# itsdevbear/go-avalanche

Measured on AMD Instinct MI355X. Metric: vote-record updates/sec (node·target·round) at 1/2/4/8 GPU; % HBM roofline, higher is better.
Workload: dtype u32; 1 GPU; C4: 1M nodes x 1000 targets, k=8, Bernoulli(0.8) initial acceptance, honest, sim mode; n_nodes=1000000, n_targets=1000, k=8, parallelism=single GPU

## Files before the change

### go-avalanche_amd/csrc/engine.cpp

```cpp
#include <algorithm>
#include <cstdarg>
#include <cstdio>
#include <cstring>
#include <memory>
#include <string>
#include <utility>
#include <vector>

#include "engine.h"

using namespace aveng;

namespace aveng {

static thread_local std::string g_last_error;

int fail(int code, const char* fmt, ...) {
  char buf[512];
  va_list ap;
  va_start(ap, fmt);
  vsnprintf(buf, sizeof(buf), fmt, ap);
  va_end(ap);
  g_last_error = buf;
  return code;
// ... 145 lines not shown
  e->log_cap = (uint32_t)std::min<size_t>(e->log_alloc / e->log_shards, 0xFFFFFFFFu);
  e->mlog_cap = (uint32_t)std::min<size_t>(e->mlog_alloc / e->log_shards, 0xFFFFFFFFu);
  e->dlog_cap = (uint32_t)std::min<size_t>(e->dlog_alloc / e->log_shards, 0xFFFFFFFFu);
}

int refresh_pref(av_engine* e) {
  e->facts.snapshot_written();
  AV_HIP(avk::launch_refresh_pref((uint32_t)e->pub_mode, e->planes, e->pref[e->cur], e->byz, (uint32_t)e->n0, e->NL,
                                  e->BL, e->PS, (uint32_t)e->round, e->stream));
  return AV_OK;
}

}

namespace {

avk::PlanShape plan_shape(const av_engine* e) {
  return {e->k,      e->BL,         e->N,               e->NL,       e->PS,
          e->capped, e->peer_world, e->comm != nullptr, e->pub_mode, e->any_nopoll};
}
avk::PlanKnobs plan_knobs(const av_engine* e) {
  return {e->kernel,   e->virtual_votes, e->vv_min_bl,     e->count_lazy,     e->k_hi_virtual,
          e->ref_rows, e->uni_rows,      e->ablate_gather, e->unsynced_shard, e->quiet_tiles != 0,
          e->net_quiet != 0, e->count_changed};
}
avk::RoundPlan plan_for(const av_engine* e, bool replay) {
  return avk::plan_round(e->facts, plan_shape(e), plan_knobs(e), replay);
}

int round_checks(const av_engine* e, int64_t rounds) {
  AV_CHECK(e->round + rounds - 1 - e->log_base < e->max_log_rounds(), AV_ERR_OVERFLOW,
           "StatusUpdate log spans %lld rounds: call av_fetch_updates more often", (long long)e->max_log_rounds());
  if (e->group) {
    AV_TRY(group_alive(e));
    for (const av_engine* m : e->group->members)
      if (m != e)
        AV_CHECK(m->round == e->round + (m->peer_rank < e->peer_rank ? 1 : 0), AV_ERR_UNSUPPORTED,
                 "peer group: rank %d at round %lld, rank %d at round %lld: run one round of every rank in rank "
                 "order", e->peer_rank, (long long)e->round, m->peer_rank, (long long)m->round);
  }
  AV_CHECK(e->NL == (uint32_t)e->N || e->comm != nullptr || e->peer_world > 1 || e->N == e->n1 - e->n0 ||
               e->unsynced_shard,
           AV_ERR_UNSUPPORTED,
           "node-sharded engine needs av_comm_init before running rounds");
  return AV_OK;
}

// ... 93 lines not shown
  }
  if (e->comm) {
    const size_t count = (size_t)e->NL * e->PS;
    uint32_t* out = e->pref[nb];
    ncclResult_t r = ncclAllGather(out + (size_t)e->n0 * e->PS, out, count, ncclUint32, e->comm, e->stream);
    AV_CHECK(r == ncclSuccess, AV_ERR_RCCL, "ncclAllGather: %s", ncclGetErrorString(r));
  }
  return AV_OK;
}

int launch_one_round(av_engine* e, const uint32_t* replay) {
  AV_TRY(round_checks(e, 1));
  avk::RoundPlan plan = plan_for(e, replay != nullptr);
  AV_CHECK(!plan.unsupported, AV_ERR_UNSUPPORTED,
           "the example responder and av_set_polling need M <= 4096 (uncapped)");
  AV_TRY(materialize(e, plan.wb_votes || plan.wb_cpreset, false));
  AV_TRY(materialize(e, false, plan.wb_counts));
  avk::RoundParams p = round_params(e, replay);
  p.c_preset = e->facts.c_preset ? 1u : 0u;
  p.vv = plan.vv ? 1u : 0u;
  p.vv_uniform = plan.vv_uniform ? 1u : 0u;
  p.fresh = plan.fresh ? 1u : 0u;
  p.klazy = plan.klazy ? 1u : 0u;
  p.kconsume = plan.kconsume ? 1u : 0u;
  p.hivirt = plan.hivirt ? 1u : 0u;
  const bool sweep = plan.kernel == avk::RoundKernel::Sweep;
  const int nb = av_engine::nxt(e->cur);
  fill_push_params(e, sweep && !replay, nb, p);
  AV_TRY(fill_row_params(e, plan, nb, p));
  if (plan.net_quiet_out) {
    p.nq_out = e->nq + (e->round & 1);
    p.nq_in = plan.net_quiet_in ? e->nq + ((e->round & 1) ^ 1) : nullptr;
    p.nq_rounds = e->nq + 2;
    p.nq_group = e->nq_group;
    p.nq_front = e->nq_front;
  }
  if (e->warm_pref && sweep) {
    if (!e->touch_sink) AV_HIP(e->touch_sink.alloc(16));
    AV_HIP(avk::launch_touch(p.pref_prev, (size_t)e->N * e->PS * 4u, e->touch_sink, e->stream));
    AV_HIP(avk::launch_touch(p.pref_in, (size_t)e->N * e->PS * 4u, e->touch_sink, e->stream));
  }
  hipEvent_t ev0 = nullptr, ev1 = nullptr;
  AV_TRY(timing_begin(e, &ev0, &ev1));
  if (p.push_n && e->masked) {
    AV_TRY(need_combine(e, e->round / avk::kNeedWin));
    AV_TRY(need_draw_ahead(e, e->round / avk::kNeedWin + 1));
// ... 377 lines not shown
constexpr PlainOption opt(const char* n, bool av_engine::*m) { return {n, kBool, 0, 1, m, nullptr, nullptr}; }
constexpr PlainOption opt(const char* n, uint32_t av_engine::*m, OptKind kd = kBool, int64_t lo = 0, int64_t hi = 1) {
  return {n, kd, lo, hi, nullptr, m, nullptr};
}
constexpr PlainOption opt(const char* n, int av_engine::*m, OptKind kd, int64_t lo, int64_t hi) {
  return {n, kd, lo, hi, nullptr, nullptr, m};
}

constexpr PlainOption kPlainOptions[] = {
    opt("plane_nt", &av_engine::plane_nt),
    opt("uniform_rows", &av_engine::uni_rows),
    opt("ref_rows", &av_engine::ref_rows),
    opt("virtual_votes", &av_engine::virtual_votes),
    opt("vv_min_bl", &av_engine::vv_min_bl, kReject, 1, (1ll << 31) - 1),
    opt("kernel", &av_engine::kernel, kReject, 1, 2),
    opt("store_policy", &av_engine::store_policy, kReject, 0, 3),
    opt("settled_fast", &av_engine::settled_fast),
    opt("settled_lean", &av_engine::settled_lean),
    opt("wave_runs", &av_engine::wave_runs),
    opt("sweep_nopipe", &av_engine::sweep_nopipe),
    opt("uni_merge", &av_engine::uni_merge, kReject, 1, 16),
    opt("uni_votes", &av_engine::uni_votes),
    opt("quiet_tiles", &av_engine::quiet_tiles),
    opt("net_quiet", &av_engine::net_quiet),
    opt("net_quiet_group", &av_engine::nq_group, kReject, 1, 16),
    opt("net_quiet_front", &av_engine::nq_front),
    opt("wave_dense", &av_engine::wave_dense, kReject, 0, 64),
    opt("tile_draw", &av_engine::tile_draw, kReject, 0, 1),
    opt("materialize_run", &av_engine::mat_run, kReject, 1, 64),
    opt("c_preset", &av_engine::c_preset),
    opt("replay_fuse", &av_engine::replay_fuse, kReject, 0, 4096),
    opt("replay_fast", &av_engine::replay_fast),
    opt("dropin_fast", &av_engine::dropin_fast),
    opt("admit_map", &av_engine::admit_map, kReject, 0, 2),
    opt("push_defer", &av_engine::push_defer),
    opt("push_store", &av_engine::push_store, kReject, 0, 2),
    opt("census_blocks", &av_engine::census_blocks, kReject, 0, 65536),
    opt("copy_blocks", &av_engine::copy_blocks, kReject, 0, 4096),
    opt("enc_buckets", &av_engine::enc_buckets, kReject, 1, 1ll << 30),
    opt("count_changed", &av_engine::count_changed),
    opt("round_marker", &av_engine::round_marker),
    opt("warm_pref", &av_engine::warm_pref),
    opt("unsynced_shard", &av_engine::unsynced_shard),
    opt("ablate_gather", &av_engine::ablate_gather),
    opt("ablate_phase", &av_engine::ablate_phase, kClamp, 0, 31),
    opt("ablate_emit", &av_engine::ablate_emit, kClamp, 0, 3),
// ... 180 lines not shown
```

### go-avalanche_amd/csrc/engine.h

```cpp
#pragma once

#include <hip/hip_runtime.h>
#include <rccl/rccl.h>

#include <algorithm>
#include <cstdint>
#include <cstdlib>
#include <thread>
#include <utility>
#include <vector>

#pragma GCC visibility push(default)
#include "../../include/avhip.h"
#pragma GCC visibility pop
#include "engine_mem.h"
#include "kernels.h"
#include "round_plan.h"

namespace aveng {
int fail(int code, const char* fmt, ...) __attribute__((format(printf, 2, 3)));
inline int oom_or_hip(hipError_t he) { return he == hipErrorOutOfMemory ? AV_ERR_OOM : AV_ERR_HIP; }
}

#define AV_HIP(call)                                                                                           \
// ... 137 lines not shown
  uint32_t mat_run = 1;
  uint32_t census_blocks = 0;
  bool masked = false;
  uint32_t segs = 1;
  avmem::DevBuf<uint8_t> need_mine;
  avmem::DevBuf<uint8_t> needmask;
  avmem::DevBuf<uint8_t> stale;
  uint32_t* needin = nullptr;
  avmem::DevBuf<uint32_t> needin_own;
  avk::PeerPtrs peer_needin{};
  int64_t need_ready = -1;
  int64_t need_pushed = -1;
  avmem::Stream need_stream;
  avmem::Event need_free, need_drawn;
  int64_t need_drawn_w = -1;
  avmem::DevBuf<unsigned long long> changed;
  bool count_changed = false;
  int64_t rflag_clear_round = 0;

  uint32_t dense_min = 0;
  uint32_t wave_dense = 0;
  uint32_t uni_votes = 1;
  uint32_t quiet_tiles = 1;
  uint32_t net_quiet = 1;
  uint32_t nq_group = 16;
  uint32_t nq_front = 1;
  avmem::DevBuf<uint32_t> nq;
  int32_t pub_mode = 0;
  avmem::DevBuf<uint32_t> readd;
  avmem::DevBuf<uint32_t> died_out;
  std::vector<uint32_t> nopoll_host;
  avmem::DevBuf<uint32_t> nopoll;
  bool any_nopoll = false;
  std::vector<int64_t> proc_round;
  avmem::DevBuf<void> fetch_scratch;
  avmem::DevBuf<unsigned long long> digest;
  avmem::PinnedBuf<void> dropin_host;
  avmem::PinnedBuf<void> stage[2];
  avmem::Event stage_ev[2];
  bool dropin_fast = true;
  uint32_t admit_map = 0;
  avmem::DevBuf<uint32_t> enc_err;
  avmem::DevBuf<uint64_t> enc_tot;
  uint32_t enc_buckets = 1u << 26;
  uint32_t copy_blocks = 0;
  static constexpr int kSlots = 3;
// ... 75 lines not shown
```

### go-avalanche_amd/csrc/kernels.h

```cpp
#pragma once

#include <hip/hip_runtime.h>
#include <stdint.h>

#include <type_traits>

namespace avk {

constexpr int kPlanes = 25;
constexpr int kPV = 0, kPC = 8, kPA = 16, kPK = 17;
constexpr uint32_t kLogShards = 1024;
constexpr uint32_t kCtrStride = 32;
constexpr uint32_t kMaxPoll = 4096;
constexpr int kMaxK = 16;
constexpr int kMaxPeers = 15;

__host__ __device__ constexpr size_t replay_groups(int k) { return (size_t)((k + 1) / 2); }
__host__ __device__ inline size_t replay_words(uint32_t Lpad, int k) { return replay_groups(k) * 4u * Lpad; }
__host__ __device__ inline size_t replay_idx(uint32_t g, int k, int j, int c) {
  return (((size_t)(g >> 6) * replay_groups(k) + (size_t)(j >> 1)) * 64u + (g & 63u)) * 4u + (size_t)((j & 1) * 2 + c);
}

__host__ __device__ constexpr uint32_t pref_stride(uint32_t BL) {
  return BL > 32u ? (BL + 31u) / 32u * 32u : (BL <= 1u ? 1u : 1u << (32 - __builtin_clz(BL - 1u)));
}

constexpr uint32_t kPendAllLive = 0x80000000u;
constexpr uint32_t kHiVirt = 0x40000000u;
__host__ __device__ inline uint32_t real_mask(uint32_t tn, uint32_t b) {
  const uint32_t rem = tn > b * 32u ? tn - b * 32u : 0u;
  return rem >= 32u ? ~0u : ((1u << rem) - 1u);
}
constexpr uint32_t kVStale = 1u, kVUniform = 2u, kVMask = 3u, kCAll = 4u;

inline void bl_divider(uint32_t d, uint32_t& magic, uint32_t& sh1, uint32_t& sh2) {
  uint32_t l = 0;
  while ((1ull << l) < d) ++l;
  magic = (uint32_t)((((1ull << l) - d) << 32) / d + 1);
  sh1 = l < 1 ? l : 1;
  sh2 = l > 1 ? l - 1 : 0;
}

__host__ __device__ constexpr uint32_t dense_words(uint32_t k) { return (k + 5u) / 2u; }
__host__ __device__ constexpr uint32_t dense_min(uint32_t k) { return dense_words(k); }

constexpr uint32_t kMedS4Died = 1u << 8;
__host__ __device__ constexpr uint32_t med_rec_words() { return 4u; }

__host__ __device__ inline uint64_t pack_update(uint32_t round_rel, uint32_t node, uint32_t slot,
                                                uint32_t target, uint32_t status, uint32_t round_shift) {
  return ((uint64_t)round_rel << round_shift) | ((uint64_t)node << 28) | ((uint64_t)slot << 24) |
         ((uint64_t)target << 2) | (uint64_t)status;
}

constexpr uint32_t kDropUnknown = 1u << 29, kDropYes = 1u << 30, kDropCons = 1u << 31, kDropTl = (1u << 22) - 1u;
__host__ __device__ inline uint32_t dropin_word(int64_t tl, bool local, uint32_t err) {
// ... 81 lines not shown

  uint32_t* uni_out;
  const uint32_t* uni_in;
  const uint32_t* uni_prev;
  uint32_t uni_world, uni_rank, uni_off;
  uint32_t uni_merge;
  uint32_t uni_post;

  uint32_t fresh;
  uint32_t tn;
  uint32_t hivirt;
  uint32_t tpw;
  uint32_t settled_fast;
  uint32_t lean;
  uint32_t bl_log2;
  uint32_t nopipe;
  uint32_t pub_mode;
  uint32_t* readd;
  uint32_t* died_out;
  const uint32_t* nopoll;
  uint32_t dense_min;
  uint32_t uni_votes;
  uint32_t quiet_tiles;
  uint32_t* nq_out;
  const uint32_t* nq_in;
  uint32_t* nq_rounds;
  uint32_t nq_group;
  uint32_t nq_front;
  uint32_t wave_dense;
  uint32_t c_preset;
};

template <int MAXK, int K = 1, typename F>
hipError_t dispatch_k(int k, F&& f) {
  if constexpr (K <= MAXK) {
    return k == K ? f(std::integral_constant<int, K>{}) : dispatch_k<MAXK, K + 1>(k, f);
  } else {
    return hipErrorInvalidValue;
  }
}

struct InitParams {
  uint32_t* planes;
  uint32_t* pref;
  const uint32_t* byz;
  uint64_t seed;
// ... 157 lines not shown
```

### go-avalanche_amd/csrc/round_plan.h

```cpp
#pragma once

#include <algorithm>
#include <cstdint>

namespace avk {

enum class RoundKernel : int {
  Sweep,
  Node,
  FirstGen,
};

enum class SweepMode : int { Replay, Ablate, Fresh, Warm, Check };

struct PlanShape {
  int k;
  uint32_t BL;
  int64_t N;
  uint32_t NL, PS;
  bool capped;
  int peer_world;
  bool has_comm;
  int32_t pub_mode;
  bool any_nopoll;
};

struct PlanKnobs {
  int kernel;
  bool virtual_votes;
  uint32_t vv_min_bl;
  bool count_lazy, k_hi_virtual, ref_rows, uni_rows, ablate_gather, unsynced_shard;
  bool quiet_tiles = true, net_quiet = true, count_changed = false;
};

struct RoundPlan {
  bool unsupported;
  RoundKernel kernel;
  SweepMode mode;
  int k;
  bool replay, capped;
  bool fresh;
  bool warm;
  bool vv;
  bool vv_uniform;
  bool klazy;
  bool kconsume;
  bool hivirt;
  bool exact_pass;
  bool wb_votes, wb_counts;
  bool wb_cpreset;
  bool ref_rows, uni_rows;
  bool net_quiet_out, net_quiet_in;
};

struct RecordFacts {
  bool c_monotone = true;
  bool warm_all = false;
  bool fresh = false;
  int count_bound = 127;
  bool c_preset = false;
  bool v_stale = false;
  bool k_pend = false;
  bool rflag_ok[3] = {false, false, false};
  bool uni_ok[3] = {false, false, false};
  bool nq_ok = false;

  void snapshot_written() {
    rflag_ok[0] = rflag_ok[1] = rflag_ok[2] = false;
    uni_ok[0] = uni_ok[1] = uni_ok[2] = false;
    nq_ok = false;
  }
  void init(bool records_created, bool preset = false) {
    snapshot_written();
    warm_all = false;
    count_bound = -6;
// ... 72 lines not shown
                                                                : RoundKernel::FirstGen;
  const bool ones = f.c_monotone && f.warm_all;
  r.fresh = f.fresh && sweep && !replay && !o.ablate_gather;
  r.warm = sweep && !replay && ones && !o.ablate_gather && !r.fresh;
  r.mode = replay            ? SweepMode::Replay
           : o.ablate_gather ? SweepMode::Ablate
           : r.fresh         ? SweepMode::Fresh
           : ones            ? SweepMode::Warm
                             : SweepMode::Check;
  r.vv = o.virtual_votes && s.k == 8 && (r.warm || r.fresh);
  r.vv_uniform = r.vv && s.BL < o.vv_min_bl;
  r.klazy = o.count_lazy && r.warm && s.k == 8 && f.count_bound < 120;
  r.kconsume = !r.klazy && f.k_pend && r.warm && s.k == 8;
  r.hivirt = o.k_hi_virtual && s.k == 8;
  r.exact_pass = f.count_bound >= 120;
  r.wb_votes = !r.vv && f.v_stale;
  r.wb_counts = !r.klazy && !r.kconsume && f.k_pend;
  r.wb_cpreset = f.c_preset && !r.fresh;
  const bool tagged = sweep && s.k == 8 && !replay && !s.has_comm && !o.ablate_gather;
  r.ref_rows = o.ref_rows && tagged && 64 % s.BL == 0;
  r.uni_rows = o.uni_rows && tagged && (s.NL == (uint32_t)s.N || s.peer_world > 1 || o.unsynced_shard);
  r.net_quiet_out = o.quiet_tiles && o.net_quiet && r.klazy && sweep && !o.count_changed && s.peer_world <= 1 && !s.has_comm;
  r.net_quiet_in = r.net_quiet_out && f.nq_ok;
  return r;
}

inline bool plans_c_preset(const PlanShape& s, const PlanKnobs& o) {
  RecordFacts f;
  f.init(true);
  const RoundPlan r = plan_round(f, s, o, false);
  return r.fresh && !r.unsupported;
}

struct SweepGrid {
  uint32_t grid, run;
};
inline SweepGrid sweep_grid(uint32_t tiles, uint32_t blocks) {
  const uint32_t need = (uint32_t)(((uint64_t)tiles + 3u) / 4u);
  const uint32_t grid = std::max(1u, blocks ? std::min(blocks, need) : need);
  const uint64_t waves = (uint64_t)grid * 4u;
  return {grid, (uint32_t)((tiles + waves - 1u) / waves)};
}
inline uint64_t sweep_run_waves(uint32_t tiles, uint32_t blocks) {
  const uint64_t run = std::max(1u, sweep_grid(tiles, blocks).run);
  return std::max<uint64_t>(1, (tiles + run - 1u) / run);
}
// ... 3 lines not shown
```

### go-avalanche_amd/csrc/round_sweep.hip

```cpp
#include <hip/hip_runtime.h>

#include <algorithm>

#include "kernels.h"
#include "round_common.h"
#include "round_plan.h"
#include "round_slots.h"

#ifndef AVK_ABLATE_PHASE
#define AVK_ABLATE_PHASE 0
#endif
#ifndef AVK_PUB_PRELOAD
#define AVK_PUB_PRELOAD 0
#endif

namespace avk {
namespace {

constexpr bool kAblatePhase = AVK_ABLATE_PHASE != 0;

struct SweepAcc {
  uint32_t applied = 0, died = 0, lane_bytes = 0;
  uint32_t reread = 0;
  uint32_t emitted_bytes = 0, updates = 0;
// ... 112 lines not shown
  uint32_t kw;
  uint32_t C[WARM ? 1 : 8];
  uint32_t uref;
  uint32_t old;
  uint32_t w[K];
  uint32_t cw[REPLAY ? K : 1];
};

struct WaveDraw {
  const uint32_t* sdc;
  const uint32_t* sdp;
  unsigned long long badc, badp;
  uint32_t fofs;
  uint32_t nlA, t0, nn;
  unsigned long long flagok;
  uint32_t meta;
  bool pair, ok;
};

__device__ __forceinline__ uint32_t meta_of(const WaveDraw& wd, uint32_t tile) {
  return (uint32_t)__builtin_amdgcn_readlane((int)wd.meta, (int)(tile - wd.t0));
}

__device__ __forceinline__ uint32_t at_byte(const uint32_t* base, uint32_t off) {
  return *reinterpret_cast<const uint32_t*>(reinterpret_cast<const char*>(base) + off);
}

struct LaneIdx {
  uint32_t g, gc, nl, b, node;
  bool active;
};

__device__ __forceinline__ LaneIdx lane_idx(const RoundParams& p, uint32_t tile, uint32_t lane) {
  LaneIdx x;
  x.g = tile * 64u + lane;
  x.active = x.g < p.L;
  x.gc = x.active ? x.g : p.L - 1u;
  x.nl = div_bl(p, x.gc);
  x.b = x.gc - x.nl * p.BL;
  x.node = p.n0 + x.nl;
  return x;
}

constexpr uint32_t kUniVotes = 1u, kUniPrev = 2u;
template <int K, bool REPLAY, bool WARM, int POL, bool ABLATE, bool VVM = false, bool FRESH = false, bool CC = true>
__device__ __forceinline__ void load_tile(const RoundParams& p, uint32_t tile, uint32_t lane,
                                          TileIn<K, REPLAY, WARM>& in, const WaveDraw* wd = nullptr,
                                          uint32_t uflags = 0u) {
  const LaneIdx x = lane_idx(p, tile, lane);
  const uint32_t* const tp = p.planes + (size_t)tile * (kPlanes * 64u);
  const u32x4* const grp = reinterpret_cast<const u32x4*>(tp) + lane;
  constexpr bool VV = VVM && WARM && !REPLAY && K == 8;
  const bool meta = VV && wd && wd->t0 <= tile && tile - wd->t0 < 64u && p.tpw;
  const uint32_t raw = VV && p.vv ? (meta ? (meta_of(*wd, tile) >> 8) & 0xFFu : uni(p.vstale[tile])) : 0u;
  in.stale = raw & kVMask;
  in.cflag = raw & kCAll;
  in.kw = 0u;
  if constexpr (FRESH) {
    const uint32_t rem = p.tn - x.b * 32u;
    const uint32_t real = rem >= 32u ? ~0u : ((1u << rem) - 1u);
    in.v0 = in.v1 = in.k0 = u32x4{0u, 0u, 0u, 0u};
    in.k1 = u32x4{0u, 0u, 0u, ~real};
#pragma unroll
    for (int i = 0; i < (WARM ? 1 : 8); ++i) in.C[i] = 0u;
  } else {
    if (!in.stale) {
      in.v0 = ld4<POL>(grp);
      in.v1 = ld4<POL>(grp + 64);
    }
    if constexpr (VV) {
      if (p.klazy || p.kconsume) in.kw = meta ? meta_of(*wd, tile) & (kPendAllLive | kHiVirt | 0xFFu) : uni(p.kpend[tile]);
    }
    if (kAblatePhase && VV && (p.ablate_phase & 2u)) {
      in.k0 = u32x4{lane, 0u, 0u, 0u};
      in.k1 = u32x4{0u, 0u, 0u, ~real_mask(p.tn, x.b)};
    } else if (!(in.kw & kPendAllLive) || !p.klazy) {
      in.k0 = ld4<POL>(grp + 128);
      if (in.kw & kHiVirt)
        in.k1 = u32x4{0u, 0u, 0u, ~real_mask(p.tn, x.b)};
// ... 78 lines not shown
#pragma unroll
    for (int j = 0; j < K; ++j) in.w[j] = at_byte(p.pref_in, rows[j] + bo);
  }
}

__device__ __forceinline__ uint8_t ref_tag(uint32_t snapshot_round) { return (uint8_t)(0x80u | (snapshot_round & 0x7Fu)); }

__device__ __forceinline__ void ref_flag_store(const RoundParams& p, uint32_t lane, bool active, uint32_t b,
                                               uint32_t node, uint32_t pub, uint32_t ref) {
  const uint64_t eq = __ballot(!active || pub == ref);
  const uint32_t s0 = lane - b;
  const uint64_t seg = (p.BL >= 64u ? ~0ull : ((1ull << p.BL) - 1ull)) << (s0 & 63u);
  if (active && b == 0u) {
    const uint8_t f = (eq & seg) == seg ? ref_tag(p.round + 1u) : 0u;
    if (p.push_n && p.rflag_out[node] != f) {
      for (uint32_t r = 0; r < p.push_n; ++r)
        __hip_atomic_store(reinterpret_cast<uint8_t*>(peer_ptr(p.push_dst, r)) + p.rflag_off + node, f, __ATOMIC_RELAXED,
                           __HIP_MEMORY_SCOPE_SYSTEM);
    }
    p.rflag_out[node] = f;
  }
}

template <int K, bool REPLAY, bool WARM, int POL, bool VVM = false, bool REF = false, bool CC = true>
__device__ __forceinline__ void process_tile(const RoundParams& p, uint32_t tile, uint32_t lane,
                                             const TileIn<K, REPLAY, WARM>& in, uint32_t extra_bytes, SweepAcc& acc,
                                             uint32_t uflags = 0u) {
  const LaneIdx x = lane_idx(p, tile, lane);
  const bool active = x.active;
  const uint32_t b = x.b, node = x.node;
  const bool nbyz = ((in.byzw >> (node & 31u)) & 1u) != 0u;
  uint32_t* const tp = p.planes + (size_t)tile * (kPlanes * 64u);
  u32x4* const grp = reinterpret_cast<u32x4*>(tp) + lane;
  const __amdgpu_buffer_rsrc_t tr = __builtin_amdgcn_make_buffer_rsrc(tp, 0, kPlanes * 64 * 4, kRsrcWord3);
  const u32x4 v0 = in.v0, v1 = in.v1;
  u32x4 k0 = in.k0, k1 = in.k1;
  uint32_t A = in.A;
  uint32_t C[8];
#pragma unroll
  for (int i = 0; i < 8; ++i) C[i] = WARM ? ~0u : in.C[WARM ? 0 : i];
  const uint32_t vmask = in.vmask;

  constexpr bool SYM = WARM && !REPLAY;
  uint32_t ys[7 + K], ns[7 + K], cwv[K];
#pragma unroll
  for (int j = 0; j < K; ++j) {
    const uint32_t cw = REPLAY ? in.cw[REPLAY ? j : 0] : ~0u;
// ... 72 lines not shown
    for (int i = 0; i < 4; ++i) {
      const uint32_t bi = ((pend >> i) & 1u) ? P0 : 0u;
      const uint32_t t = Kp[3 + i] ^ bi;
      const uint32_t si = t ^ cy;
      cy = (t & cy) | (Kp[3 + i] & bi);
      Kp[3 + i] = si;
    }
  }
  uint32_t E[K], alive = P0, applied = 0u, c[4] = {0u, 0u, 0u, 0u}, F = 0u;
  const uint32_t low3[3] = {Kp[0], Kp[1], Kp[2]};
  constexpr bool KLZ_ABLATE = VVM && WARM && !REPLAY && K == 8;
  const uint32_t nearfin = klazy ? 0u : P0 & Kp[6] & Kp[5] & Kp[4] & Kp[3];
  const bool det = __ballot(nearfin != 0u) != 0ull;
  const uint32_t A_in = A;
  bool settled = false;
  if constexpr (SYM && K == 8) {
    if (!det) {
      uint32_t agree = P0;
#pragma unroll
      for (int i = 0; i < 7 + K; ++i) agree &= ~(ys[i] ^ A);
      settled = __ballot(agree != P0) == 0ull;
    }
  }
  if (settled) {
#pragma unroll
    for (int j = 0; j < K; ++j) E[j] = 0u;
    c[3] = P0;
    applied = 8u * (uint32_t)__popc(P0);
  } else if (kAblatePhase && KLZ_ABLATE && (p.ablate_phase & 16u)) {
#pragma unroll
    for (int j = 0; j < K; ++j) E[j] = 0u;
    c[3] = P0;
    applied = 8u * (uint32_t)__popc(P0);
  } else {
    round_slots<K, SYM>(ys, ns, low3, nearfin, det, alive, A, E, c, F, applied);
  }
  bool kdefer = false;
  uint32_t pend = 0u;
  if constexpr (KL) {
    if (klazy) {
      const uint32_t c8 = c[3] & ~(c[0] | c[1] | c[2]);
      const bool lane_uniform = !active || (((F & P0) | (~c8 & P0)) == 0u);
      kdefer = __ballot(!lane_uniform) == 0ull;
      pend = in.kw & 0xFFu;
      if (!kdefer) {
        if (kunread) {
          k0 = ld4<POL>(reinterpret_cast<const u32x4*>(tp) + lane + 128);
          k1 = in.kw & kHiVirt ? u32x4{0u, 0u, 0u, ~real_mask(p.tn, b)}
                               : ld4<POL>(reinterpret_cast<const u32x4*>(tp) + lane + 192);
#pragma unroll
          for (int i = 0; i < 4; ++i) {
            Kp[i] = k0[i];
            Kp[4 + i] = k1[i];
          }
        }
        uint32_t cy = 0u;
#pragma unroll
        for (int i = 0; i < 4; ++i) {
          const uint32_t bi = ((pend >> i) & 1u) ? P0 : 0u;
// ... 31 lines not shown
    if (AVK_PUB_PRELOAD && CC && p.count_changed && !known) pre = publish_loads(p, node * p.PS + b, node - p.n0);
    if (!kdefer) {
      u32x4 o2, o3;
#pragma unroll
      for (int i = 0; i < 4; ++i) {
        o2[i] = Kp[i];
        o3[i] = Kp[4 + i];
      }
      st4<POL>(tr, grp + 128, 2048u + lane * 16u, o2);
      if (!hv) st4<POL>(tr, grp + 192, 3072u + lane * 16u, o3);
    }
    if (astore) st1<POL>(tr, tp + 1536u + lane, (1536u + lane) * 4u, A);
    const uint32_t prow = node * p.PS + b;
    const uint32_t pub = nbyz ? byz_pattern(p.round + 1u) : A;
    if (p.uni_out) acc.umis |= pub != in.uref ? 1u : 0u;
    publish<POL, CC>(p, prow, pub, nbyz ? byz_pattern(p.round - 2u) : pub, acc, known, node - p.n0, acc.qslot, &pre);
  }
  if (REF && p.rflag_out && settled) {
    ref_flag_store(p, lane, active, b, node, nbyz ? byz_pattern(p.round + 1u) : A,
                   p.pref_in[p.ref_node * p.PS + (active ? b : 0u)]);
    if (active) acc.lane_bytes += 4u + (b == 0u ? 1u : 0u);
  }
  if constexpr (VVM && !REPLAY && K == 8) {
    const uint32_t nv = (virt ? (settled ? kVUniform : kVStale) : 0u) | in.cflag | (cvirt && !p.c_preset ? kCAll : 0u);
    if (p.vv && lane == 0 && nv != (in.stale | in.cflag)) p.vstale[tile] = nv;
  }
  if constexpr (KL) {
    if (klazy) {
      const bool all_live = __ballot(active && live0 != vmask) == 0ull;
      const uint32_t kw = (kdefer ? pend + 1u : 0u) | (all_live ? kPendAllLive : 0u) | (hv ? kHiVirt : 0u);
      if (lane == 0 && kw != in.kw) p.kpend[tile] = kw;
      if (lane == 0) acc.lane_bytes += kw != in.kw ? 8u : 4u;
    } else if (kcons) {
      if (lane == 0 && in.kw) p.kpend[tile] = 0u;
      if (lane == 0) acc.lane_bytes += in.kw ? 8u : 4u;
    }
  }
  if constexpr (!WARM && !REPLAY && K == 8) {
    if (hv && lane == 0) {
      p.kpend[tile] = kHiVirt;
      acc.lane_bytes += 4u;
    }
  }
  uint32_t emitted;
  if constexpr (K == 8)
    emitted = emit_store_med<K>(p, acc.shard, lane, node, p.t0 + b * 32u, E, A, died, er, p.round_rel);
  else
    emitted = emit_updates<K>(p, tile, lane, node, p.t0 + b * 32u, E, A, died, acc.updates);

  constexpr uint32_t plane_bytes = WARM ? 2u * 17u * 4u : 2u * kPlanes * 4u;
  const uint32_t lane_bytes = plane_bytes + (REPLAY ? 8u : 4u) * K + 4u - (!WARM && p.fresh ? 96u : 0u);
  acc.applied += applied;
  acc.died += (uint32_t)__popc(died);
  const uint32_t kbytes = (kunread && kdefer ? 32u : 0u) + (kdefer ? 32u : 0u) +
                          (WARM && (in.kw & kHiVirt) && !(kunread && kdefer) ? 16u : 0u) + (hv && !kdefer ? 16u : 0u);
  acc.lane_bytes += active ? lane_bytes + extra_bytes - (in.stale == kVStale ? 4u : in.stale == kVUniform ? 32u : 0u) -
                                 (virt ? 32u : 0u) - (cvirt ? 32u : 0u) + (p.count_changed ? 4u : 0u) -
                                 kbytes - (astore ? 0u : 4u) - ((uflags & kUniVotes) ? 4u * K - 4u : 0u) -
                                 (in.stale == kVStale && (uflags & kUniPrev) ? 24u : 0u)
                           : 0u;
  acc.emitted_bytes += emitted;
  if constexpr (!REPLAY)
    acc.reread += active ? ((uflags & kUniVotes) ? 4u : 4u * K - 4u) +
                               (in.stale == kVStale ? ((uflags & kUniPrev) ? 4u : 24u) : 0u)
                         : 0u;
}

template <int POL, bool REF, bool CC>
__device__ __forceinline__ bool settled_tile(const RoundParams& p, uint32_t tile, uint32_t lane, uint32_t kw,
                                             const WaveDraw& wd, SweepAcc& acc) {
  const uint32_t g = tile * 64u + lane;
  const bool active = g < p.L;
  const uint32_t gc = active ? g : p.L - 1u;
  const uint32_t nl = div_bl(p, gc);
  const uint32_t b = gc - nl * p.BL;
  const __amdgpu_buffer_rsrc_t ta =
      __builtin_amdgcn_make_buffer_rsrc(p.planes + (size_t)tile * (kPlanes * 64u), 0, kPlanes * 64 * 4, kRsrcWord3);
  const uint32_t A = __builtin_amdgcn_raw_buffer_load_b32(ta, (1536u + lane) * 4u, 0, POL > 0 ? 2 : 0);
  const uint32_t P0 = active ? at_byte(p.valid, b * 4u) : 0u;
  const uint32_t uref = p.uni_out ? p.pref_in[p.ref_node * p.PS + b] : 0u;
  uint32_t rows[8];
  pick_parked(p, wd.sdc, wd.badc, (nl - wd.nlA) * 2u, p.n0 + nl, p.round, p.PS * 4u, rows);
  const uint32_t bo = b * 4u;
  uint32_t dis = 0u, all = ~0u;
  bool gather = true;
  uint32_t rbytes = 0u;
  if (REF && p.rflag_in) {
    const uint32_t rw = p.pref_prev[p.ref_node * p.PS + b];
    uint32_t fl = 1u;
#pragma unroll
    for (int j = 0; j < 8; ++j) fl &= p.rflag_in[rows[j] >> p.ps_shift] == ref_tag(p.round) ? 1u : 0u;
    rbytes = 4u + (b == 0u ? 8u : 0u);
    if (fl) {
      dis = all = rw;
      gather = false;
    }
  }
  if (gather) {
#pragma unroll
    for (int j = 0; j < 8; ++j) dis |= at_byte(p.pref_in, rows[j] + bo);
#pragma unroll
    for (int j = 0; j < 8; ++j) all &= at_byte(p.pref_in, rows[j] + bo);
  }
  if (__ballot(((dis ^ A) | (all ^ A)) & P0) != 0ull) return false;
  const uint32_t node = p.n0 + nl;
  const uint32_t pub = is_byz(p.byz, node) ? byz_pattern(p.round + 1u) : A;
  if (active) {
    if (p.uni_out) acc.umis |= pub != uref ? 1u : 0u;
    const uint32_t prow = node * p.PS + b;
    const bool known = (kw & 0xFFu) >= 2u;
    publish<POL, CC>(p, prow, pub, is_byz(p.byz, node) ? byz_pattern(p.round - 2u) : pub, acc, known, nl, acc.qslot);
  }
  if (REF && p.rflag_out) ref_flag_store(p, lane, active, b, node, pub, p.pref_in[p.ref_node * p.PS + (active ? b : 0u)]);
  if (lane == 0) p.kpend[tile] = ((kw & 0xFFu) + 1u) | kPendAllLive | (kw & kHiVirt);
  acc.applied += 8u * (uint32_t)__popc(P0);
  acc.reread += active && gather ? 28u : 0u;
  acc.lane_bytes += (active ? 40u + (p.count_changed ? 4u : 0u) + rbytes - (gather ? 0u : 32u) +
                                  (REF && p.rflag_out ? 4u + (b == 0u ? 1u : 0u) : 0u)
                            : 0u) +
                    (lane == 0 ? 8u : 0u);
  return true;
}

template <int POL, bool REF, bool CC>
__device__ __forceinline__ uint32_t settled_run(const RoundParams& p, uint32_t lane, uint32_t tile_end,
                                                const WaveDraw& wd, SweepAcc& acc) {
  const uint32_t t0 = wd.t0, ntiles = tile_end - t0;
  const uint32_t b = lane & (p.BL - 1u), bo = b * 4u;
  const uint32_t vw = at_byte(p.valid, bo);
  const unsigned long long byzm = __ballot(lane < wd.nn && is_byz(p.byz, p.n0 + wd.nlA + lane));
  const uint32_t bpat = byz_pattern(p.round + 1u);
  const __amdgpu_buffer_rsrc_t ta =
      __builtin_amdgcn_make_buffer_rsrc(p.planes + (size_t)t0 * (kPlanes * 64u), 0, (int)(ntiles * kPlanes * 64u * 4u),
                                        kRsrcWord3);
  const uint32_t aoff = (1536u + lane) * 4u;
  const bool rd = REF && p.rflag_in && wd.flagok != 0ull;
  const uint32_t rprev = rd ? at_byte(p.pref_prev, p.ref_node * p.PS * 4u + bo) : 0u;
  const uint32_t rin = (REF && p.rflag_out) || p.uni_out ? at_byte(p.pref_in, p.ref_node * p.PS * 4u + bo) : 0u;
  uint32_t done = 0u, umis = 0u;
  uint32_t applied = 0u, bytes = 0u, reread = 0u;
  for (uint32_t i = 0; i < ntiles; ++i) {
    const uint32_t m = (uint32_t)__builtin_amdgcn_readlane((int)wd.meta, (int)i);
    if ((m & (kPendAllLive | (kVMask << 8))) != (kPendAllLive | (kVUniform << 8))) continue;
    const uint32_t tile = t0 + i;
    const uint32_t A = __builtin_amdgcn_raw_buffer_load_b32(ta, aoff + i * (kPlanes * 64u * 4u), 0, POL > 0 ? 2 : 0);
    const uint32_t g = tile * 64u + lane;
    const bool active = g < p.L;
    const uint32_t nl = (active ? g : p.L - 1u) >> p.bl_log2;
    const uint32_t P0 = active ? vw : 0u;
    const uint32_t rel = nl - wd.nlA;
    uint32_t rows[8];
    {
      const uint32_t* q = wd.sdc + rel * 8u;
      const u32x4 lo = *reinterpret_cast<const u32x4*>(q);
      const u32x4 hi = *reinterpret_cast<const u32x4*>(q + 4);
#pragma unroll
      for (int c = 0; c < 4; ++c) {
        rows[c] = lo[c];
        rows[c + 4] = hi[c];
      }
    }
    uint32_t dis = 0u, all = ~0u;
    bool gather = true;
    if (rd) {
      const uint32_t base = rel * 2u + wd.fofs;
      const bool fl = ((wd.flagok >> base) & 3ull) == 3ull;
// ... 10 lines not shown
        all &= w;
      }
    }
    if (__ballot(((dis ^ A) | (all ^ A)) & P0) != 0ull) continue;
    const uint32_t node = p.n0 + nl;
    const uint32_t pub = ((byzm >> rel) & 1ull) ? bpat : A;
    if (active) {
      umis |= pub != rin ? 1u : 0u;
      const uint32_t prow = node * p.PS + b;
      const bool known = (m & 0xFFu) >= 2u;
      publish<POL, CC>(p, prow, pub, ((byzm >> rel) & 1ull) ? byz_pattern(p.round - 2u) : pub, acc, known, nl, i);
    }
    if (REF && p.rflag_out) ref_flag_store(p, lane, active, b, node, pub, rin);
    done |= 1u << i;
    applied += 8u * (uint32_t)__popc(P0);
    bytes += active ? 40u + (p.count_changed ? 4u : 0u) - (gather ? 0u : 32u) +
                          (REF && p.rflag_out ? (b == 0u ? 1u : 0u) : 0u)
                    : 0u;
    reread += active && gather ? 28u : 0u;
  }
  if (lane < ntiles && ((done >> lane) & 1u)) {
    p.kpend[t0 + lane] = ((wd.meta & 0xFFu) + 1u) | kPendAllLive | (wd.meta & kHiVirt);
    bytes += 8u;
  }
  acc.applied += applied;
  acc.lane_bytes += bytes;
  acc.reread += reread;
  if (p.uni_out) acc.umis |= umis;
  return done;
}

constexpr uint32_t kUniRun = 16;

struct UniPre {
  uint32_t Av[kUniRun];
  uint32_t vw, refp, rin;
  uint32_t bz[4];
  unsigned long long byzm[4];
};

__device__ __forceinline__ void uni_early(const RoundParams& p, uint32_t lane, uint32_t nlA, UniPre& u) {
  u.vw = at_byte(p.valid, (lane & (p.BL - 1u)) * 4u);
#pragma unroll
  for (uint32_t j = 0; j < 4u; ++j)
    u.bz[j] = is_byz(p.byz, min(p.n0 + nlA + lane + 64u * j, p.n_nodes - 1u)) ? 1u : 0u;
}
// ... 25 lines not shown

template <int POL, bool CC>
__device__ __forceinline__ uint32_t settled_run_uni(const RoundParams& p, uint32_t lane, uint32_t t0,
                                                    uint32_t tile_end, uint32_t meta, uint32_t nlA, uint32_t nn,
                                                    const UniPre& u, uint32_t quiet, SweepAcc& acc) {
  const uint32_t ntiles = tile_end - t0;
  const uint32_t b = lane & (p.BL - 1u);
  const uint32_t vw = u.vw, refp = u.refp, rin = u.rin;
  if ((u.byzm[0] | u.byzm[1] | u.byzm[2] | u.byzm[3]) != 0ull) return 0u;
  if constexpr (!CC) {
    if (quiet) {
      const bool mine = lane < ntiles && ((quiet >> lane) & 1u);
      if (mine) p.kpend[t0 + lane] = ((meta & 0xFFu) + 1u) | kPendAllLive | (meta & kHiVirt);
      const uint32_t last = (p.Lpad >> 6) - 1u;
      const bool cut = last < tile_end && ((quiet >> (last - t0)) & 1u) && last * 64u + lane >= p.L;
      acc.applied += 8u * (uint32_t)__popc(vw) * ((uint32_t)__popc(quiet) - (cut ? 1u : 0u));
      acc.lane_bytes += mine ? 8u : 0u;
      if (quiet == (uint32_t)((1ull << ntiles) - 1ull)) return quiet;
    }
  }
  uint32_t cand = 0u;
  for (uint32_t i = 0; i < ntiles; ++i) {
    const uint32_t m = (uint32_t)__builtin_amdgcn_readlane((int)meta, (int)i);
    if ((m & (kPendAllLive | (kVMask << 8))) == (kPendAllLive | (kVUniform << 8))) cand |= 1u << i;
  }
  cand &= ~quiet;
  uint32_t Av[kUniRun];
#pragma unroll
  for (uint32_t i = 0; i < kUniRun; ++i) Av[i] = u.Av[i];
  if constexpr (!CC) {
    const __amdgpu_buffer_rsrc_t prb =
        __builtin_amdgcn_make_buffer_rsrc(p.pref_out, 0, (int)(p.n_nodes * p.PS * 4u), kRsrcWord3);
    uint32_t done = 0u, applied = 0u, bytes = 0u, umis = 0u;
    const uint32_t npt = 64u >> p.bl_log2;
    const uint32_t rel0 = ((t0 * 64u + lane) >> p.bl_log2) - nlA;
    uint32_t prow = (p.n0 + nlA + rel0) * p.PS + b;
#pragma unroll
    for (uint32_t i = 0; i < kUniRun; ++i) {
      const uint32_t g = (t0 + i) * 64u + lane;
      const bool active = g < p.L;
      const uint32_t P0 = active ? vw : 0u;
      const uint32_t A = Av[i];
      const uint32_t mis = __ballot((refp ^ A) & P0) != 0ull ? 1u : 0u;
      const bool ok = (((cand >> i) & 1u) & (mis ^ 1u)) != 0u;
      const uint32_t pub = A;
      const bool st = ok && active;
      __builtin_amdgcn_raw_buffer_store_b32(pub, prb, st ? prow * 4u : 0xFFFFFFFCu, 0, POL == 1 ? 2 : 0);
      umis |= (st & (pub != rin)) ? 1u : 0u;
      done |= ok ? 1u << i : 0u;
      applied += st ? 8u * (uint32_t)__popc(P0) : 0u;
      bytes += st ? 8u : 0u;
      prow += npt * p.PS;
    }
    if (lane < ntiles && ((done >> lane) & 1u)) {
      p.kpend[t0 + lane] = ((meta & 0xFFu) + 1u) | kPendAllLive | (meta & kHiVirt);
      bytes += 8u;
    }
    acc.applied += applied;
    acc.lane_bytes += bytes;
    if (p.uni_out) acc.umis |= umis;
    return done | quiet;
  }
  uint32_t done = 0u, applied = 0u, bytes = 0u, umis = 0u;
#pragma unroll
  for (uint32_t i = 0; i < kUniRun; ++i) {
    if (!((cand >> i) & 1u)) continue;
    const uint32_t tile = t0 + i;
    const uint32_t A = Av[i];
    const uint32_t g = tile * 64u + lane;
    const bool active = g < p.L;
    const uint32_t nl = (active ? g : p.L - 1u) >> p.bl_log2;
    const uint32_t P0 = active ? vw : 0u;
    if (__ballot((refp ^ A) & P0) != 0ull) continue;
    const uint32_t node = p.n0 + nl;
    const uint32_t pub = A;
    if (active) {
      umis |= pub != rin ? 1u : 0u;
      const uint32_t prow = node * p.PS + b;
      const uint32_t m = (uint32_t)__builtin_amdgcn_readlane((int)meta, (int)i);
      const bool known = (m & 0xFFu) >= 2u;
      publish<POL, CC>(p, prow, pub, pub, acc, known, nl, i);
    }
    done |= 1u << i;
    applied += 8u * (uint32_t)__popc(P0);
    bytes += active ? 8u + (p.count_changed ? 4u : 0u) : 0u;
  }
  if (lane < ntiles && ((done >> lane) & 1u)) {
    p.kpend[t0 + lane] = ((meta & 0xFFu) + 1u) | kPendAllLive | (meta & kHiVirt);
    bytes += 8u;
  }
  acc.applied += applied;
  acc.lane_bytes += bytes;
  if (p.uni_out) acc.umis |= umis;
  return done;
}

constexpr uint32_t kNqChunks = 4;
__device__ __forceinline__ void net_quiet_run(const RoundParams& p, uint32_t lane, uint32_t t0, uint32_t tile_end,
                                              SweepAcc& acc) {
  const uint32_t n = tile_end - t0;
  const uint32_t vw = at_byte(p.valid, (lane & (p.BL - 1u)) * 4u);
  uint32_t kw[kNqChunks];
#pragma unroll
  for (uint32_t c = 0; c < kNqChunks; ++c) kw[c] = c * 64u + lane < n ? p.kpend[t0 + c * 64u + lane] : 0u;
  uint32_t mine = 0u;
#pragma unroll
  for (uint32_t c = 0; c < kNqChunks; ++c) {
    if (c * 64u + lane < n) {
      p.kpend[t0 + c * 64u + lane] = ((kw[c] & 0xFFu) + 1u) | kPendAllLive | (kw[c] & kHiVirt);
      ++mine;
    }
  }
// ... 90 lines not shown
          const uint32_t nn = nlB - nlA + 1u;
          UniPre upre;
          const bool uni_ok = p.uni_in && p.lean && p.settled_fast && p.klazy && p.vv && nn <= 256u &&
                              tile_end - tile <= kUniRun;
          const uint32_t ti = tile + lane;
          const uint32_t st = p.vv && ti < tile_end ? p.vstale[ti] : 0u;
          const uint32_t kw = (p.klazy || p.kconsume) && ti < tile_end ? p.kpend[ti] : 0u;
          if constexpr (!CC) {
            if (uni_ok) uni_early(p, lane, nlA, upre);
          }
          wd.meta = (st << 8) | (kw & (kPendAllLive | kHiVirt | 0xFFu));
          wd.t0 = tile;
          wd.nlA = nlA;
          wd.nn = nn;
          const uint32_t all_tiles = (uint32_t)((1ull << (tile_end - tile)) - 1ull);
          if (uni_ok && uniform) {
            const bool qt = !CC && prev_uni && p.quiet_tiles;
            if constexpr (CC) uni_early(p, lane, nlA, upre);
            const uint32_t quiet = uni_prefetch<POL>(p, lane, tile, tile_end, nn, wd.meta, qt, upre);
            uni_done = settled_run_uni<POL, CC>(p, lane, tile, tile_end, wd.meta, nlA, nn, upre, quiet, acc);
            uni_ran = true;
            if (quiet == all_tiles && uni_done == all_tiles) nq_tag = false;
          }
          const bool any_stale = __ballot((st & kVMask) == kVStale) != 0ull;
          if (uni_done != all_tiles) {
            wd.pair = any_stale;
            wd.flagok = 0ull;
            if (any_stale && nn * 2u > 32u) {
              const PairDraw dp = single_draw(p, p.round - 1u, nlA, nn, lane);
              const PairDraw dc = single_draw(p, p.round, nlA, nn, lane);
              wd.ok = !dp.fallback && !dc.fallback;
              if (wd.ok) {
                park_draw(dp, sd, lane, p.PS * 4u);
                park_draw(dc, sd + 256, lane, p.PS * 4u);
              }
              wd.sdp = sd;
              wd.sdc = sd + 256;
              wd.badp = dp.bad;
              wd.badc = dc.bad;
            } else {
              const PairDraw d = any_stale ? pair_draw(p, p.round, nlA, nn, lane) : single_draw(p, p.round, nlA, nn, lane);
              wd.ok = !d.fallback;
              if (wd.ok) park_draw(d, sd, lane, p.PS * 4u);
              wd.sdp = sd;
              wd.sdc = any_stale ? sd + 128 : sd;
              wd.badp = d.bad & 0xFFFFFFFFull;
              wd.badc = any_stale ? d.bad >> 32 : d.bad;
// ... 37 lines not shown
        if constexpr (K == 8) {
          if (lean_done && ((lean_done >> (tile - wd.t0)) & 1u)) continue;
          if (tdraw) {
            const uint32_t tnlA = uni(div_bl(p, tile * 64u));
            const uint32_t tnn = uni(div_bl(p, min(tile * 64u + 64u, p.L) - 1u)) - tnlA + 1u;
            const bool tst = ((meta_of(wd, tile) >> 8) & kVMask) == kVStale;
            const PairDraw d = tst ? pair_draw(p, p.round, tnlA, tnn, lane) : single_draw(p, p.round, tnlA, tnn, lane);
            wd.ok = !d.fallback;
            if (wd.ok) {
              park_draw(d, sd, lane, p.PS * 4u);
              wd.nlA = tnlA;
              wd.nn = tnn;
              wd.pair = tst;
              wd.sdp = sd;
              wd.sdc = tst ? sd + 128 : sd;
              wd.badp = d.bad & 0xFFFFFFFFull;
              wd.badc = tst ? d.bad >> 32 : d.bad;
              wd.fofs = tst ? 32u : 0u;
              wd.flagok = 0ull;
            }
          }
          if (wd.ok && p.settled_fast && p.klazy && p.vv && !lean_ran) {
            const uint32_t m = meta_of(wd, tile);
            if (((m >> 8) & kVMask) == kVUniform && (m & kPendAllLive) &&
                settled_tile<POL, REF, CC>(p, tile, lane, m & (kPendAllLive | kHiVirt | 0xFFu), wd, acc))
              continue;
          }
        }
        TileIn<K, false, true> in;
        load_tile<K, false, true, POL, false, true, false, CC>(p, tile, lane, in, &wd, uflags);
        process_tile<K, false, true, POL, true, REF, CC>(p, tile, lane, in, 0u, acc, uflags);
      } else if constexpr (MODE == kModeFresh) {
        TileIn<K, false, false> in;
        load_tile<K, false, false, POL, false, true, true>(p, tile, lane, in);
        process_tile<K, false, false, POL, true>(p, tile, lane, in, 0u, acc);
      } else if constexpr (MODE == kModeReplay) {
        TileIn<K, true, false> in;
        load_tile<K, true, false, POL, false>(p, tile, lane, in);
        process_tile<K, true, false, POL>(p, tile, lane, in, 0u, acc);
      } else {
        bool warm = false;
        if (p.warm_skip) {
          const uint32_t g = tile * 64u + lane;
          const uint32_t c7 = g < p.L ? p.planes[(size_t)tile * (kPlanes * 64u) + 1024u + 7u * 64u + lane] : ~0u;
          warm = __all(c7 == ~0u);
        }
        if (warm) {
          TileIn<K, false, true> in;
          load_tile<K, false, true, POL, AB>(p, tile, lane, in);
          process_tile<K, false, true, POL>(p, tile, lane, in, 4u, acc);
        } else {
          TileIn<K, false, false> in;
          load_tile<K, false, false, POL, AB>(p, tile, lane, in);
          process_tile<K, false, false, POL>(p, tile, lane, in, 0u, acc);
// ... 235 lines not shown
```

Before: 32530 billion vote-record updates/s (1 update = 1 regsiterVote on a live record; k=8 per node·target·round).

## Add calm-tile tag so stale tiles with settled history take the fast settle path

```diff
diff --git a/go-avalanche_amd/csrc/engine.cpp b/go-avalanche_amd/csrc/engine.cpp
--- a/go-avalanche_amd/csrc/engine.cpp
+++ b/go-avalanche_amd/csrc/engine.cpp
@@ -191,7 +191,7 @@
 avk::PlanKnobs plan_knobs(const av_engine* e) {
   return {e->kernel,   e->virtual_votes, e->vv_min_bl,     e->count_lazy,     e->k_hi_virtual,
           e->ref_rows, e->uni_rows,      e->ablate_gather, e->unsynced_shard, e->quiet_tiles != 0,
-          e->net_quiet != 0, e->count_changed};
+          e->net_quiet != 0, e->count_changed, e->calm_tiles != 0};
 }
 avk::RoundPlan plan_for(const av_engine* e, bool replay) {
   return avk::plan_round(e->facts, plan_shape(e), plan_knobs(e), replay);
@@ -331,6 +331,7 @@
   p.vv_uniform = plan.vv_uniform ? 1u : 0u;
   p.fresh = plan.fresh ? 1u : 0u;
   p.klazy = plan.klazy ? 1u : 0u;
+  p.calm = plan.calm ? 1u : 0u;
   p.kconsume = plan.kconsume ? 1u : 0u;
   p.hivirt = plan.hivirt ? 1u : 0u;
   const bool sweep = plan.kernel == avk::RoundKernel::Sweep;
@@ -754,6 +755,7 @@
     opt("uni_merge", &av_engine::uni_merge, kReject, 1, 16),
     opt("uni_votes", &av_engine::uni_votes),
     opt("quiet_tiles", &av_engine::quiet_tiles),
+    opt("calm_tiles", &av_engine::calm_tiles),
     opt("net_quiet", &av_engine::net_quiet),
     opt("net_quiet_group", &av_engine::nq_group, kReject, 1, 16),
     opt("net_quiet_front", &av_engine::nq_front),
diff --git a/go-avalanche_amd/csrc/engine.h b/go-avalanche_amd/csrc/engine.h
--- a/go-avalanche_amd/csrc/engine.h
+++ b/go-avalanche_amd/csrc/engine.h
@@ -183,6 +183,7 @@
   uint32_t wave_dense = 0;
   uint32_t uni_votes = 1;
   uint32_t quiet_tiles = 1;
+  uint32_t calm_tiles = 1;
   uint32_t net_quiet = 1;
   uint32_t nq_group = 16;
   uint32_t nq_front = 1;
diff --git a/go-avalanche_amd/csrc/kernels.h b/go-avalanche_amd/csrc/kernels.h
--- a/go-avalanche_amd/csrc/kernels.h
+++ b/go-avalanche_amd/csrc/kernels.h
@@ -32,6 +32,7 @@
   return rem >= 32u ? ~0u : ((1u << rem) - 1u);
 }
 constexpr uint32_t kVStale = 1u, kVUniform = 2u, kVMask = 3u, kCAll = 4u;
+constexpr uint32_t kVCalm = 8u;
 
 inline void bl_divider(uint32_t d, uint32_t& magic, uint32_t& sh1, uint32_t& sh2) {
   uint32_t l = 0;
@@ -159,6 +160,7 @@
   uint32_t dense_min;
   uint32_t uni_votes;
   uint32_t quiet_tiles;
+  uint32_t calm;
   uint32_t* nq_out;
   const uint32_t* nq_in;
   uint32_t* nq_rounds;
diff --git a/go-avalanche_amd/csrc/round_plan.h b/go-avalanche_amd/csrc/round_plan.h
--- a/go-avalanche_amd/csrc/round_plan.h
+++ b/go-avalanche_amd/csrc/round_plan.h
@@ -31,6 +31,7 @@
   uint32_t vv_min_bl;
   bool count_lazy, k_hi_virtual, ref_rows, uni_rows, ablate_gather, unsynced_shard;
   bool quiet_tiles = true, net_quiet = true, count_changed = false;
+  bool calm_tiles = true;
 };
 
 struct RoundPlan {
@@ -51,6 +52,7 @@
   bool wb_cpreset;
   bool ref_rows, uni_rows;
   bool net_quiet_out, net_quiet_in;
+  bool calm;
 };
 
 struct RecordFacts {
@@ -169,6 +171,7 @@
   r.uni_rows = o.uni_rows && tagged && (s.NL == (uint32_t)s.N || s.peer_world > 1 || o.unsynced_shard);
   r.net_quiet_out = o.quiet_tiles && o.net_quiet && r.klazy && sweep && !o.count_changed && s.peer_world <= 1 && !s.has_comm;
   r.net_quiet_in = r.net_quiet_out && f.nq_ok;
+  r.calm = o.calm_tiles && r.klazy && r.vv && !r.vv_uniform && s.k == 8 && sweep;
   return r;
 }
 
diff --git a/go-avalanche_amd/csrc/round_sweep.hip b/go-avalanche_amd/csrc/round_sweep.hip
--- a/go-avalanche_amd/csrc/round_sweep.hip
+++ b/go-avalanche_amd/csrc/round_sweep.hip
@@ -158,6 +158,16 @@
   return (uint32_t)__builtin_amdgcn_readlane((int)wd.meta, (int)(tile - wd.t0));
 }
 
+__device__ __forceinline__ bool settled_cand(uint32_t m, uint32_t calm) {
+  const uint32_t v = (m >> 8) & (kVMask | kVCalm);
+  return (m & kPendAllLive) && (v == kVUniform || (calm && v == (kVStale | kVCalm)));
+}
+__device__ __forceinline__ uint32_t calm_settle(const RoundParams& p, uint32_t tile, uint32_t m) {
+  if (!((m >> 8) & kVCalm)) return 0u;
+  p.vstale[tile] = kVUniform | ((m >> 8) & kCAll);
+  return 4u;
+}
+
 __device__ __forceinline__ uint32_t at_byte(const uint32_t* base, uint32_t off) {
   return *reinterpret_cast<const uint32_t*>(reinterpret_cast<const char*>(base) + off);
 }
@@ -190,7 +200,7 @@
   const bool meta = VV && wd && wd->t0 <= tile && tile - wd->t0 < 64u && p.tpw;
   const uint32_t raw = VV && p.vv ? (meta ? (meta_of(*wd, tile) >> 8) & 0xFFu : uni(p.vstale[tile])) : 0u;
   in.stale = raw & kVMask;
-  in.cflag = raw & kCAll;
+  in.cflag = raw & (kCAll | kVCalm);
   in.kw = 0u;
   if constexpr (FRESH) {
     const uint32_t rem = p.tn - x.b * 32u;
@@ -315,7 +325,7 @@
   }
 }
 
-template <int K, bool REPLAY, bool WARM, int POL, bool VVM = false, bool REF = false, bool CC = true>
+template <int K, bool REPLAY, bool WARM, int POL, bool VVM = false, bool REF = false, bool CC = true, bool CALM = false>
 __device__ __forceinline__ void process_tile(const RoundParams& p, uint32_t tile, uint32_t lane,
                                              const TileIn<K, REPLAY, WARM>& in, uint32_t extra_bytes, SweepAcc& acc,
                                              uint32_t uflags = 0u) {
@@ -434,6 +444,15 @@
       settled = __ballot(agree != P0) == 0ull;
     }
   }
+  bool calm_pre = false;
+  if constexpr (CALM && KL && SYM) {
+    if (p.calm && klazy && virt && !settled && __ballot(((ys[8] ^ A) & (ys[9] ^ A) & P0) != 0u) == 0ull) {
+      Agg2 g{~(ys[8] ^ A), ~0u};
+#pragma unroll
+      for (int j = 2; j < 8; ++j) agg_push(g, ~(ys[7 + j] ^ A));
+      calm_pre = __ballot((~g.z1 & P0) != 0u) == 0ull;
+    }
+  }
   if (settled) {
 #pragma unroll
     for (int j = 0; j < K; ++j) E[j] = 0u;
@@ -447,6 +466,7 @@
   } else {
     round_slots<K, SYM>(ys, ns, low3, nearfin, det, alive, A, E, c, F, applied);
   }
+  const bool calm = calm_pre && __ballot((F & P0) != 0u) == 0ull;
   bool kdefer = false;
   uint32_t pend = 0u;
   if constexpr (KL) {
@@ -524,7 +544,8 @@
     if (active) acc.lane_bytes += 4u + (b == 0u ? 1u : 0u);
   }
   if constexpr (VVM && !REPLAY && K == 8) {
-    const uint32_t nv = (virt ? (settled ? kVUniform : kVStale) : 0u) | in.cflag | (cvirt && !p.c_preset ? kCAll : 0u);
+    const uint32_t nv = (virt ? (settled ? kVUniform : kVStale) : 0u) | (in.cflag & kCAll) |
+                        (cvirt && !p.c_preset ? kCAll : 0u) | (calm ? kVCalm : 0u);
     if (p.vv && lane == 0 && nv != (in.stale | in.cflag)) p.vstale[tile] = nv;
   }
   if constexpr (KL) {
@@ -570,7 +591,7 @@
 
 template <int POL, bool REF, bool CC>
 __device__ __forceinline__ bool settled_tile(const RoundParams& p, uint32_t tile, uint32_t lane, uint32_t kw,
-                                             const WaveDraw& wd, SweepAcc& acc) {
+                                             const WaveDraw& wd, SweepAcc& acc, uint32_t vst) {
   const uint32_t g = tile * 64u + lane;
   const bool active = g < p.L;
   const uint32_t gc = active ? g : p.L - 1u;
@@ -615,12 +636,13 @@
   }
   if (REF && p.rflag_out) ref_flag_store(p, lane, active, b, node, pub, p.pref_in[p.ref_node * p.PS + (active ? b : 0u)]);
   if (lane == 0) p.kpend[tile] = ((kw & 0xFFu) + 1u) | kPendAllLive | (kw & kHiVirt);
+  const uint32_t cbytes = lane == 0 ? calm_settle(p, tile, vst << 8) : 0u;
   acc.applied += 8u * (uint32_t)__popc(P0);
   acc.reread += active && gather ? 28u : 0u;
   acc.lane_bytes += (active ? 40u + (p.count_changed ? 4u : 0u) + rbytes - (gather ? 0u : 32u) +
                                   (REF && p.rflag_out ? 4u + (b == 0u ? 1u : 0u) : 0u)
                             : 0u) +
-                    (lane == 0 ? 8u : 0u);
+                    (lane == 0 ? 8u : 0u) + cbytes;
   return true;
 }
 
@@ -643,7 +665,7 @@
   uint32_t applied = 0u, bytes = 0u, reread = 0u;
   for (uint32_t i = 0; i < ntiles; ++i) {
     const uint32_t m = (uint32_t)__builtin_amdgcn_readlane((int)wd.meta, (int)i);
-    if ((m & (kPendAllLive | (kVMask << 8))) != (kPendAllLive | (kVUniform << 8))) continue;
+    if (!settled_cand(m, byzm ? 0u : p.calm)) continue;
     const uint32_t tile = t0 + i;
     const uint32_t A = __builtin_amdgcn_raw_buffer_load_b32(ta, aoff + i * (kPlanes * 64u * 4u), 0, POL > 0 ? 2 : 0);
     const uint32_t g = tile * 64u + lane;
@@ -700,6 +722,7 @@
   if (lane < ntiles && ((done >> lane) & 1u)) {
     p.kpend[t0 + lane] = ((wd.meta & 0xFFu) + 1u) | kPendAllLive | (wd.meta & kHiVirt);
     bytes += 8u;
+    bytes += calm_settle(p, t0 + lane, wd.meta);
   }
   acc.applied += applied;
   acc.lane_bytes += bytes;
@@ -771,7 +794,7 @@
   uint32_t cand = 0u;
   for (uint32_t i = 0; i < ntiles; ++i) {
     const uint32_t m = (uint32_t)__builtin_amdgcn_readlane((int)meta, (int)i);
-    if ((m & (kPendAllLive | (kVMask << 8))) == (kPendAllLive | (kVUniform << 8))) cand |= 1u << i;
+    if (settled_cand(m, p.calm)) cand |= 1u << i;
   }
   cand &= ~quiet;
   uint32_t Av[kUniRun];
@@ -804,6 +827,7 @@
     if (lane < ntiles && ((done >> lane) & 1u)) {
       p.kpend[t0 + lane] = ((meta & 0xFFu) + 1u) | kPendAllLive | (meta & kHiVirt);
       bytes += 8u;
+      bytes += calm_settle(p, t0 + lane, meta);
     }
     acc.applied += applied;
     acc.lane_bytes += bytes;
@@ -837,6 +861,7 @@
   if (lane < ntiles && ((done >> lane) & 1u)) {
     p.kpend[t0 + lane] = ((meta & 0xFFu) + 1u) | kPendAllLive | (meta & kHiVirt);
     bytes += 8u;
+    bytes += calm_settle(p, t0 + lane, meta);
   }
   acc.applied += applied;
   acc.lane_bytes += bytes;
@@ -973,7 +998,7 @@
             uni_ran = true;
             if (quiet == all_tiles && uni_done == all_tiles) nq_tag = false;
           }
-          const bool any_stale = __ballot((st & kVMask) == kVStale) != 0ull;
+          const bool any_stale = __ballot((st & kVMask) == kVStale && lane < 32u && !((uni_done >> lane) & 1u)) != 0ull;
           if (uni_done != all_tiles) {
             wd.pair = any_stale;
             wd.flagok = 0ull;
@@ -1057,14 +1082,16 @@
           }
           if (wd.ok && p.settled_fast && p.klazy && p.vv && !lean_ran) {
             const uint32_t m = meta_of(wd, tile);
-            if (((m >> 8) & kVMask) == kVUniform && (m & kPendAllLive) &&
-                settled_tile<POL, REF, CC>(p, tile, lane, m & (kPendAllLive | kHiVirt | 0xFFu), wd, acc))
+            const bool cok = p.calm && ((m >> 8) & kVCalm) &&
+                             __ballot(lane < wd.nn && is_byz(p.byz, p.n0 + wd.nlA + lane)) == 0ull;
+            if (settled_cand(m, cok ? 1u : 0u) &&
+                settled_tile<POL, REF, CC>(p, tile, lane, m & (kPendAllLive | kHiVirt | 0xFFu), wd, acc, m >> 8))
               continue;
           }
         }
         TileIn<K, false, true> in;
         load_tile<K, false, true, POL, false, true, false, CC>(p, tile, lane, in, &wd, uflags);
-        process_tile<K, false, true, POL, true, REF, CC>(p, tile, lane, in, 0u, acc, uflags);
+        process_tile<K, false, true, POL, true, REF, CC, true>(p, tile, lane, in, 0u, acc, uflags);
       } else if constexpr (MODE == kModeFresh) {
         TileIn<K, false, false> in;
         load_tile<K, false, false, POL, false, true, true>(p, tile, lane, in);
```

Result: faster. 35810 billion vote-record updates/s (1 update = 1 regsiterVote on a live record; k=8 per node·target·round), median of 6 (+10.1%).
